# William-gregory/SeaIceExtentForecasting

Hardware: NVIDIA B200
Metric: retrospective forecasts/sec (network+GPR) (higher is better)
Workload: dtype f64

## Files before the change

### seaiceextentforecasting_b200/csrc/gp.cu

```cuda
#include "common.cuh"

namespace {

constexpr int GT = 256;
constexpr int MAXN = 64;
constexpr int LDS = MAXN + 1;

__device__ const double kTheta[5] = {1.495585217958292e-002, 2.539398330063230e-001, 9.504178996162932e-001,
                                     2.097847961257068e+000, 4.25};
__device__ const double kCoeff[5] = {1.1102230246251565e-16 * 100800.0, 1.1102230246251565e-16 * 10059033600.0,
                                     1.1102230246251565e-16 * 4487938430976000.0,
                                     1.1102230246251565e-16 * 5914384781877411840000.0,
                                     1.1102230246251565e-16 * 113250775606021113483283660800000000.0};
__device__ const double kB3[4] = {120., 60., 12., 1.};
__device__ const double kB5[6] = {30240., 15120., 3360., 420., 30., 1.};
__device__ const double kB7[8] = {17297280., 8648640., 1995840., 277200., 25200., 1512., 56., 1.};
__device__ const double kB9[10] = {17643225600., 8821612800., 2075673600., 302702400., 30270240.,
                                   2162160., 110880., 3960., 90., 1.};
__device__ const double kB13[14] = {64764752532480000., 32382376266240000., 7771770303897600., 1187353796428800.,
                                    129060195264000., 10559470521600., 670442572800., 33522128640., 1323241920.,
                                    40840800., 960960., 16380., 182., 1.};

__device__ unsigned long long g_gp_phase[16];
#ifdef SIE_GP_TIMERS
#define GP_TICK(i) do { if (threadIdx.x == 0) { const long long t__ = clock64(); atomicAdd(&g_gp_phase[i], (unsigned long long)(t__ - gp_t_last)); gp_t_last = t__; } } while (0)
#else
#define GP_TICK(i) do { } while (0)
#endif
constexpr int KC = 16;
constexpr int LDA_S = 20;
constexpr int LDB_S = 68;
constexpr int PANEL = 16;

struct Smem {
  double As[2][64 * LDA_S];
  double Bs[2][KC * LDB_S];
  union {
    struct {
      double K[MAXN * LDS];
      double W[MAXN * LDS];
    } gp;
    double panel[2 * MAXN * LDS];
  } u;
  double y[MAXN], ya[MAXN], alpha[MAXN], kxs[MAXN], v[MAXN];
  double red[GT / 32];
  int ired[GT / 32];
  int misc[8];
  double dmisc[8];
  int piv[PANEL];
};

__device__ __forceinline__ double block_sum(double v, Smem& sm) {
#pragma unroll
  for (int o = 16; o > 0; o >>= 1) v += __shfl_xor_sync(0xffffffffu, v, o);
  __syncthreads();
  if ((threadIdx.x & 31) == 0) sm.red[threadIdx.x >> 5] = v;
  __syncthreads();
  double r = 0.0;
#pragma unroll
  for (int w = 0; w < GT / 32; ++w) r += sm.red[w];
  return r;
}
__device__ __forceinline__ double block_max(double v, Smem& sm) {
#pragma unroll
  for (int o = 16; o > 0; o >>= 1) v = fmax(v, __shfl_xor_sync(0xffffffffu, v, o));
  __syncthreads();
  if ((threadIdx.x & 31) == 0) sm.red[threadIdx.x >> 5] = v;
  __syncthreads();
  double r = sm.red[0];
#pragma unroll
  for (int w = 1; w < GT / 32; ++w) r = fmax(r, sm.red[w]);
  return r;
}

__device__ __forceinline__ void dmma884(double& c0, double& c1, double a, double b) {
  asm volatile("mma.sync.aligned.m8n8k4.row.col.f64.f64.f64.f64 {%0,%1}, {%2}, {%3}, {%0,%1};"
               : "+d"(c0), "+d"(c1)
               : "d"(a), "d"(b));
}

__device__ __noinline__ void cta_gemm(double* __restrict__ Cm, int ldc, const double* __restrict__ A, int lda,
                         const double* __restrict__ Bm, int ldb, int m, int k, int n2, Smem& sm, int mode = 0) {
  if (m <= 0 || n2 <= 0 || k <= 0) { __syncthreads(); return; }
  const int tid = threadIdx.x, lane = tid & 31, warp = tid >> 5;
  const int wr = warp >> 1, wc = warp & 1;
  const int tm = (m + 63) >> 6, tn = (n2 + 63) >> 6, kc = (k + KC - 1) / KC;
  const int nsteps = tm * tn * kc;
  const int ar = tid >> 2, ak = (tid & 3) * 4;
  const int bk = tid >> 4, bc = (tid & 15) * 4;
  double ra[4], rb[4];
  auto gload = [&](int step) {
    const int t = step / kc, c = step - t * kc;
    const int ti = t / tn, tj = t - ti * tn;
    const int gr = ti * 64 + ar, gk = c * KC + ak;
    const double* pa = A + (size_t)gr * lda + gk;
#pragma unroll
    for (int q = 0; q < 4; ++q) ra[q] = (gr < m && gk + q < k) ? pa[q] : 0.0;
    const int gkb = c * KC + bk, gc = tj * 64 + bc;
    const double* pb = Bm + (size_t)gkb * ldb + gc;
#pragma unroll
    for (int q = 0; q < 4; ++q) rb[q] = (gkb < k && gc + q < n2) ? pb[q] : 0.0;
  };
  auto spark = [&](int bufi) {
    double* as = sm.As[bufi] + ar * LDA_S + ak;
    double* bs = sm.Bs[bufi] + bk * LDB_S + bc;
    *reinterpret_cast<double2*>(as) = make_double2(ra[0], ra[1]);
    *reinterpret_cast<double2*>(as + 2) = make_double2(ra[2], ra[3]);
    *reinterpret_cast<double2*>(bs) = make_double2(rb[0], rb[1]);
    *reinterpret_cast<double2*>(bs + 2) = make_double2(rb[2], rb[3]);
  };
  double acc[2][4][2];
  gload(0);
  spark(0);
  __syncthreads();
  for (int step = 0; step < nsteps; ++step) {
    const int bufi = step & 1;
    const int t = step / kc, c = step - t * kc;
    if (step + 1 < nsteps) gload(step + 1);
    if (c == 0) {
#pragma unroll
      for (int i = 0; i < 2; ++i)
#pragma unroll
        for (int jj = 0; jj < 4; ++jj) acc[i][jj][0] = acc[i][jj][1] = 0.0;
    }
    const double* as = sm.As[bufi] + (wr * 16 + (lane >> 2)) * LDA_S + (lane & 3);
    const double* bs = sm.Bs[bufi] + (lane & 3) * LDB_S + wc * 32 + (lane >> 2);
#pragma unroll
    for (int ks = 0; ks < KC / 4; ++ks) {
      double af[2], bf[4];
#pragma unroll
      for (int i = 0; i < 2; ++i) af[i] = as[i * 8 * LDA_S + ks * 4];
#pragma unroll
      for (int jj = 0; jj < 4; ++jj) bf[jj] = bs[ks * 4 * LDB_S + jj * 8];
#pragma unroll
      for (int i = 0; i < 2; ++i)
#pragma unroll
        for (int jj = 0; jj < 4; ++jj) dmma884(acc[i][jj][0], acc[i][jj][1], af[i], bf[jj]);
    }
    if (c == kc - 1) {
      const int ti = t / tn, tj = t - ti * tn;
#pragma unroll
      for (int i = 0; i < 2; ++i) {
        const int gr = ti * 64 + wr * 16 + i * 8 + (lane >> 2);
        if (gr >= m) continue;
#pragma unroll
        for (int jj = 0; jj < 4; ++jj) {
          const int gc = tj * 64 + wc * 32 + jj * 8 + 2 * (lane & 3);
          double* pc = Cm + (size_t)gr * ldc + gc;
          if (gc < n2) pc[0] = mode ? pc[0] - acc[i][jj][0] : acc[i][jj][0];
          if (gc + 1 < n2) pc[1] = mode ? pc[1] - acc[i][jj][1] : acc[i][jj][1];
        }
      }
    }
    if (step + 1 < nsteps) spark(bufi ^ 1);
    __syncthreads();
  }
}

__device__ __noinline__ double cta_norm1(const double* __restrict__ A, int ld, int np_, Smem& sm) {
  double best = 0.0;
  for (int j = threadIdx.x; j < np_; j += GT) {
    double s = 0.0;
    for (int i = 0; i < np_; ++i) s += fabs(A[(size_t)i * ld + j]);
    best = fmax(best, s);
  }
  return block_max(best, sm);
}

__device__ __noinline__ double cta_absnorm_power(const double* __restrict__ A, int ld, int np_, double scale, int p,
                                    double* __restrict__ v0, double* __restrict__ v1, Smem& sm) {
  const int parts = (np_ <= GT / 8) ? 8 : (np_ <= GT / 4) ? 4 : (np_ <= GT / 2) ? 2 : 1;
  double* part = &sm.As[0][0];
  const int jc = threadIdx.x % np_, sl = threadIdx.x / np_;
  for (int j = threadIdx.x; j < np_; j += GT) v0[j] = 1.0;
  __syncthreads();
  double* src = v0;
  double* dst = v1;
  for (int it = 0; it < p; ++it) {
    if (parts > 1) {
      if (sl < parts) {
        double s = 0.0;
#pragma unroll 4
        for (int i = sl; i < np_; i += parts) s = fma(scale * fabs(A[(size_t)i * ld + jc]), src[i], s);
        part[sl * np_ + jc] = s;
      }
      __syncthreads();
      if (threadIdx.x < np_) {
        double s = part[threadIdx.x];
        for (int q = 1; q < parts; ++q) s += part[q * np_ + threadIdx.x];
        dst[threadIdx.x] = s;
      }
    } else {
      for (int j = threadIdx.x; j < np_; j += GT) {
        double s = 0.0;
#pragma unroll 4
        for (int i = 0; i < np_; ++i) s = fma(scale * fabs(A[(size_t)i * ld + j]), src[i], s);
        dst[j] = s;
      }
    }
    __syncthreads();
    double* t = src; src = dst; dst = t;
  }
  double best = 0.0;
  for (int j = threadIdx.x; j < np_; j += GT) best = fmax(best, src[j]);
  return block_max(best, sm);
}

__device__ __forceinline__ int ell_of(double t, double normA, int idx, int m) {
  if (!(t > 0.0)) return 0;
  const double val = ceil(log2(t / normA / kCoeff[idx]) / (double)(2 * m));
  if (val != val) return 1 << 20;
  if (val > 1.0e6) return 1 << 20;
  return val > 0.0 ? (int)val : 0;
}

__device__ __noinline__ void cta_lincomb(double* __restrict__ dst, int ld, int np_, double cI, const double* P1, double c1,
                            const double* P2, double c2, const double* P3, double c3, const double* add) {
#pragma unroll 4
  for (int idx = threadIdx.x; idx < np_ * np_; idx += GT) {
    const int i = idx / np_, jj = idx - i * np_;
    const size_t o = (size_t)i * ld + jj;
    double v = (i == jj) ? cI : 0.0;
    if (P1) v += c1 * P1[o];
    if (P2) v += c2 * P2[o];
    if (P3) v += c3 * P3[o];
    if (add) v += add[o];
    dst[o] = v;
  }
  __syncthreads();
}

__device__ __noinline__ void cta_lu_solve(double* __restrict__ P, double* __restrict__ Q, int ld, int np_, Smem& sm) {
  const int tid = threadIdx.x;
  double* pan = sm.u.panel;
  for (int k0 = 0; k0 < np_; k0 += PANEL) {
    const int kb = min(PANEL, np_ - k0);
    const int rows = np_ - k0;
    for (int idx = tid; idx < rows * PANEL; idx += GT) {
      const int r = idx / PANEL, c = idx - r * PANEL;
      pan[idx] = (c < kb) ? P[(size_t)(k0 + r) * ld + k0 + c] : 0.0;
    }
    __syncthreads();
    for (int c = 0; c < kb; ++c) {
      double bv = -1.0; int bi = c;
      for (int r = c + tid; r < rows; r += GT) {
        const double a = fabs(pan[r * PANEL + c]);
        if (a > bv) { bv = a; bi = r; }
      }
#pragma unroll
      for (int o = 16; o > 0; o >>= 1) {
        const double ov = __shfl_xor_sync(0xffffffffu, bv, o);
        const int oi = __shfl_xor_sync(0xffffffffu, bi, o);
        if (ov > bv || (ov == bv && oi < bi)) { bv = ov; bi = oi; }
      }
      if ((tid & 31) == 0) { sm.red[tid >> 5] = bv; sm.ired[tid >> 5] = bi; }
      __syncthreads();
      bv = sm.red[0]; bi = sm.ired[0];
#pragma unroll
      for (int w = 1; w < GT / 32; ++w)
        if (sm.red[w] > bv || (sm.red[w] == bv && sm.ired[w] < bi)) { bv = sm.red[w]; bi = sm.ired[w]; }
      if (tid == 0) sm.piv[c] = bi;
      if (bi != c && tid < PANEL) {
        const double t = pan[c * PANEL + tid]; pan[c * PANEL + tid] = pan[bi * PANEL + tid]; pan[bi * PANEL + tid] = t;
      }
      __syncthreads();
      const double inv = 1.0 / pan[c * PANEL + c];
      for (int r = c + 1 + tid; r < rows; r += GT) pan[r * PANEL + c] *= inv;
      __syncthreads();
      const int cw = kb - c - 1;
      if (cw > 0) {
        for (int idx = tid; idx < (rows - c - 1) * cw; idx += GT) {
          const int r = c + 1 + idx / cw, c2 = c + 1 + idx % cw;
          pan[r * PANEL + c2] = fma(-pan[r * PANEL + c], pan[c * PANEL + c2], pan[r * PANEL + c2]);
        }
      }
      __syncthreads();
    }
    for (int idx = tid; idx < rows * kb; idx += GT) {
      const int r = idx / kb, c = idx - r * kb;
      P[(size_t)(k0 + r) * ld + k0 + c] = pan[r * PANEL + c];
    }
    const int rightw = np_ - k0 - kb;
    for (int col = tid; col < rightw + np_; col += GT) {
      double* base = (col < rightw) ? P + (k0 + kb + col) : Q + (col - rightw);
      for (int c = 0; c < kb; ++c) {
        const int pr = sm.piv[c];
        if (pr != c) {
          const double t = base[(size_t)(k0 + c) * ld]; base[(size_t)(k0 + c) * ld] = base[(size_t)(k0 + pr) * ld];
          base[(size_t)(k0 + pr) * ld] = t;
        }
      }
      double x[PANEL];
#pragma unroll
      for (int c = 0; c < PANEL; ++c) x[c] = (c < kb) ? base[(size_t)(k0 + c) * ld] : 0.0;
#pragma unroll
      for (int c = 1; c < PANEL; ++c) {
        if (c < kb) {
          double sacc = x[c];
#pragma unroll
          for (int d = 0; d < PANEL; ++d)
            if (d < c) sacc = fma(-pan[c * PANEL + d], x[d], sacc);
          x[c] = sacc;
        }
      }
#pragma unroll
      for (int c = 0; c < PANEL; ++c)
        if (c < kb) base[(size_t)(k0 + c) * ld] = x[c];
    }
    __syncthreads();
    const int below = np_ - k0 - kb;
    if (below > 0) {
      const double* L21 = P + (size_t)(k0 + kb) * ld + k0;
      cta_gemm(P + (size_t)(k0 + kb) * ld + k0 + kb, ld, L21, ld, P + (size_t)k0 * ld + k0 + kb, ld, below, kb, rightw,
               sm, 1);
      cta_gemm(Q + (size_t)(k0 + kb) * ld, ld, L21, ld, Q + (size_t)k0 * ld, ld, below, kb, np_, sm, 1);
    }
  }
  const int nblk = (np_ + PANEL - 1) / PANEL;
  for (int b = nblk - 1; b >= 0; --b) {
    const int k0 = b * PANEL, kb = min(PANEL, np_ - k0);
    for (int idx = tid; idx < PANEL * PANEL; idx += GT) {
      const int r = idx / PANEL, c = idx - r * PANEL;
      pan[idx] = (r < kb && c < kb) ? P[(size_t)(k0 + r) * ld + k0 + c] : 0.0;
    }
    __syncthreads();
    for (int col = tid; col < np_; col += GT) {
      double x[PANEL];
#pragma unroll
      for (int c = 0; c < PANEL; ++c) x[c] = (c < kb) ? Q[(size_t)(k0 + c) * ld + col] : 0.0;
#pragma unroll
      for (int c = PANEL - 1; c >= 0; --c) {
        if (c < kb) {
          double sacc = x[c];
#pragma unroll
          for (int d = 0; d < PANEL; ++d)
            if (d > c && d < kb) sacc = fma(-pan[c * PANEL + d], x[d], sacc);
          x[c] = sacc / pan[c * PANEL + c];
        }
      }
#pragma unroll
      for (int c = 0; c < PANEL; ++c)
        if (c < kb) Q[(size_t)(k0 + c) * ld + col] = x[c];
    }
    __syncthreads();
    if (k0 > 0) cta_gemm(Q, ld, P + k0, ld, Q + (size_t)k0 * ld, ld, k0, kb, np_, sm, 1);
  }
}

__device__ __noinline__ double* cta_expm(double** buf, int ld, int np_, double* v0, double* v1, int* m_out, int* s_out,
                            Smem& sm) {
  double* A = buf[1]; double* A2 = buf[2]; double* A4 = buf[3]; double* A6 = buf[4];
  double* B5 = buf[5]; double* B6 = buf[6]; double* B7 = buf[7]; double* B8 = buf[8];
  long long gp_t_last = clock64();
  (void)gp_t_last;
  cta_gemm(A2, ld, A, ld, A, ld, np_, np_, np_, sm);
  cta_gemm(A4, ld, A2, ld, A2, ld, np_, np_, np_, sm);
  cta_gemm(A6, ld, A4, ld, A2, ld, np_, np_, np_, sm);
  const double normA = cta_norm1(A, ld, np_, sm);
  const double d4 = pow(cta_norm1(A4, ld, np_, sm), 0.25);
  const double d6 = pow(cta_norm1(A6, ld, np_, sm), 1.0 / 6.0);
  const double eta0 = fmax(d4, d6);
  GP_TICK(1);
  int m = 0, s = 0;
  if (eta0 < kTheta[0] && ell_of(cta_absnorm_power(A, ld, np_, 1.0, 7, v0, v1, sm), normA, 0, 3) == 0) m = 3;
  if (!m && eta0 < kTheta[1] && ell_of(cta_absnorm_power(A, ld, np_, 1.0, 11, v0, v1, sm), normA, 1, 5) == 0) m = 5;
  double d8 = 0.0, eta2 = 0.0;
  if (!m) {
    cta_gemm(B5, ld, A4, ld, A4, ld, np_, np_, np_, sm);
    d8 = pow(cta_norm1(B5, ld, np_, sm), 0.125);
    eta2 = fmax(d6, d8);
    if (eta2 < kTheta[2] && ell_of(cta_absnorm_power(A, ld, np_, 1.0, 15, v0, v1, sm), normA, 2, 7) == 0) m = 7;
    if (!m && eta2 < kTheta[3] && ell_of(cta_absnorm_power(A, ld, np_, 1.0, 19, v0, v1, sm), normA, 3, 9) == 0) m = 9;
  }
  GP_TICK(2);
  double* U = B7; double* V = B8;
  if (m == 3) {
    cta_lincomb(B5, ld, np_, kB3[1], A2, kB3[3], nullptr, 0, nullptr, 0, nullptr);
    cta_gemm(U, ld, A, ld, B5, ld, np_, np_, np_, sm);
    cta_lincomb(V, ld, np_, kB3[0], A2, kB3[2], nullptr, 0, nullptr, 0, nullptr);
  } else if (m == 5) {
    cta_lincomb(B5, ld, np_, kB5[1], A4, kB5[5], A2, kB5[3], nullptr, 0, nullptr);
    cta_gemm(U, ld, A, ld, B5, ld, np_, np_, np_, sm);
    cta_lincomb(V, ld, np_, kB5[0], A4, kB5[4], A2, kB5[2], nullptr, 0, nullptr);
  } else if (m == 7) {
    cta_lincomb(B5, ld, np_, kB7[1], A6, kB7[7], A4, kB7[5], A2, kB7[3], nullptr);
    cta_gemm(U, ld, A, ld, B5, ld, np_, np_, np_, sm);
    cta_lincomb(V, ld, np_, kB7[0], A6, kB7[6], A4, kB7[4], A2, kB7[2], nullptr);
  } else if (m == 9) {
    cta_lincomb(B6, ld, np_, kB9[1], A6, kB9[7], A4, kB9[5], A2, kB9[3], nullptr);
    for (int idx = threadIdx.x; idx < np_ * np_; idx += GT) {
      const int i = idx / np_, jj = idx - i * np_; const size_t o = (size_t)i * ld + jj;
      B6[o] += kB9[9] * B5[o];
    }
    __syncthreads();
    cta_gemm(U, ld, A, ld, B6, ld, np_, np_, np_, sm);
    cta_lincomb(V, ld, np_, kB9[0], A6, kB9[6], A4, kB9[4], A2, kB9[2], nullptr);
    for (int idx = threadIdx.x; idx < np_ * np_; idx += GT) {
      const int i = idx / np_, jj = idx - i * np_; const size_t o = (size_t)i * ld + jj;
      V[o] += kB9[8] * B5[o];
    }
    __syncthreads();
  } else {
    m = 13;
    cta_gemm(B6, ld, A4, ld, A6, ld, np_, np_, np_, sm);
    const double d10 = pow(cta_norm1(B6, ld, np_, sm), 0.1);
    const double eta3 = fmax(d8, d10), eta4 = fmin(eta2, eta3);
    double sv = ceil(log2(eta4 / kTheta[4]));
    s = (sv > 0.0) ? (int)sv : 0;
    if (!(sv == sv) || sv > 2000.0) s = 2000;
    const double sc = ldexp(1.0, -s);
    GP_TICK(2);
    s += ell_of(cta_absnorm_power(A, ld, np_, sc, 27, v0, v1, sm), normA * sc, 4, 13);
    GP_TICK(3);
    if (s > 2000) s = 2000;
    const double s1 = ldexp(1.0, -s), s2 = ldexp(1.0, -2 * s), s4 = ldexp(1.0, -4 * s), s6 = ldexp(1.0, -6 * s);
#pragma unroll 2
    for (int idx = threadIdx.x; idx < np_ * np_; idx += GT) {
      const int i = idx / np_, jj = idx - i * np_; const size_t o = (size_t)i * ld + jj;
      A[o] *= s1; A2[o] *= s2; A4[o] *= s4; A6[o] *= s6;
    }
    __syncthreads();
    cta_lincomb(B5, ld, np_, 0.0, A6, kB13[13], A4, kB13[11], A2, kB13[9], nullptr);
    cta_gemm(B6, ld, A6, ld, B5, ld, np_, np_, np_, sm);
    cta_lincomb(B5, ld, np_, kB13[1], A6, kB13[7], A4, kB13[5], A2, kB13[3], B6);
    cta_gemm(U, ld, A, ld, B5, ld, np_, np_, np_, sm);
    cta_lincomb(B5, ld, np_, 0.0, A6, kB13[12], A4, kB13[10], A2, kB13[8], nullptr);
    cta_gemm(B6, ld, A6, ld, B5, ld, np_, np_, np_, sm);
    cta_lincomb(V, ld, np_, kB13[0], A6, kB13[6], A4, kB13[4], A2, kB13[2], B6);
  }
  GP_TICK(4);
#pragma unroll 4
  for (int idx = threadIdx.x; idx < np_ * np_; idx += GT) {
    const int i = idx / np_, jj = idx - i * np_; const size_t o = (size_t)i * ld + jj;
    const double u = U[o], vv = V[o];
    B5[o] = vv - u; B6[o] = vv + u;
  }
  __syncthreads();
  cta_lu_solve(B5, B6, ld, np_, sm);
  GP_TICK(5);
  double* Xc = B6; double* Xn = B7;
  for (int it = 0; it < s; ++it) {
    cta_gemm(Xn, ld, Xc, ld, Xc, ld, np_, np_, np_, sm);
    double* t = Xc; Xc = Xn; Xn = t;
  }
  GP_TICK(6);
  *m_out = m; *s_out = s;
  return Xc;
}

__device__ __noinline__ int cta_cholesky(double* K, int n, Smem& sm) {
  const int tid = threadIdx.x;
  for (int k = 0; k < n; ++k) {
    const double d = K[k * LDS + k];
    if (!(d > 0.0)) return k + 1;
    const double r = sqrt(d);
    __syncthreads();
    if (tid == 0) K[k * LDS + k] = r;
    for (int i = k + 1 + tid; i < n; i += GT) K[i * LDS + k] /= r;
    __syncthreads();
    const int rem = n - k - 1;
    for (int idx = tid; idx < rem * rem; idx += GT) {
      const int a = idx / rem, b = idx - a * rem;
      if (b <= a) {
        const int i = k + 1 + a, jj = k + 1 + b;
        K[i * LDS + jj] = fma(-K[i * LDS + k], K[jj * LDS + k], K[i * LDS + jj]);
      }
    }
    __syncthreads();
  }
  return 0;
}
__device__ __forceinline__ void warp_fwd_solve(const double* L, int n, const double* b, double* tmp, int lane) {
  for (int i = 0; i < n; ++i) {
    double s = 0.0;
    for (int c = lane; c < i; c += 32) s = fma(L[i * LDS + c], tmp[c], s);
#pragma unroll
    for (int o = 16; o > 0; o >>= 1) s += __shfl_xor_sync(0xffffffffu, s, o);
    if (lane == 0) tmp[i] = (b[i] - s) / L[i * LDS + i];
    __syncwarp();
  }
}
__device__ __forceinline__ void warp_bwd_solve(const double* L, int n, const double* tmp, double* x, int lane) {
  for (int i = n - 1; i >= 0; --i) {
    double s = 0.0;
    for (int c = i + 1 + lane; c < n; c += 32) s = fma(L[c * LDS + i], x[c], s);
#pragma unroll
    for (int o = 16; o > 0; o >>= 1) s += __shfl_xor_sync(0xffffffffu, s, o);
    if (lane == 0) x[i] = (tmp[i] - s) / L[i * LDS + i];
    __syncwarp();
  }
}
__device__ void cta_chol_solve(const double* L, int n, const double* b, double* x, double* tmp) {
  if (threadIdx.x < 32) {
    warp_fwd_solve(L, n, b, tmp, threadIdx.x);
    warp_bwd_solve(L, n, tmp, x, threadIdx.x);
  }
  __syncthreads();
}

__device__ __forceinline__ int warp_cholesky(double* K, int n, int ldw, int lane) {
  for (int k = 0; k < n; ++k) {
    const double d = K[k * ldw + k];
    if (!(d > 0.0)) return k + 1;
    const double r = sqrt(d);
    __syncwarp();
    if (lane == 0) K[k * ldw + k] = r;
    for (int i = k + 1 + lane; i < n; i += 32) K[i * ldw + k] /= r;
    __syncwarp();
    for (int i = k + 1 + lane; i < n; i += 32) {
      const double aik = K[i * ldw + k];
      for (int jj = k + 1; jj <= i; ++jj) K[i * ldw + jj] = fma(-aik, K[jj * ldw + k], K[i * ldw + jj]);
    }
    __syncwarp();
  }
  return 0;
}
__device__ __forceinline__ void warp_fwd_solve_ld(const double* L, int n, int ldw, const double* b, double* tmp, int lane) {
  for (int i = 0; i < n; ++i) {
    double s = 0.0;
    for (int c = lane; c < i; c += 32) s = fma(L[i * ldw + c], tmp[c], s);
#pragma unroll
    for (int o = 16; o > 0; o >>= 1) s += __shfl_xor_sync(0xffffffffu, s, o);
    if (lane == 0) tmp[i] = (b[i] - s) / L[i * ldw + i];
    __syncwarp();
  }
}
__device__ __forceinline__ void warp_bwd_solve_ld(const double* L, int n, int ldw, const double* tmp, double* x, int lane) {
  for (int i = n - 1; i >= 0; --i) {
    double s = 0.0;
    for (int c = i + 1 + lane; c < n; c += 32) s = fma(L[c * ldw + i], x[c], s);
#pragma unroll
    for (int o = 16; o > 0; o >>= 1) s += __shfl_xor_sync(0xffffffffu, s, o);
    if (lane == 0) x[i] = (tmp[i] - s) / L[i * ldw + i];
    __syncwarp();
  }
}

__device__ void warp_sigma_fit(const double* __restrict__ W, const double* __restrict__ y, const double* __restrict__ kxs_raw,
                               double kss_raw, const double* __restrict__ G1raw, int n, double sig, double* Kw, double* vec,
                               SieGpResult& res, long long clk_start, SieGpResult* outp) {
  const int lane = threadIdx.x & 31;
  const int ldw = n | 1;
  double* ya = vec; double* alpha = vec + MAXN; double* kxs = vec + 2 * MAXN; double* v = vec + 3 * MAXN;
  res.fmean = res.fvar = res.sigma_f = res.nlml = res.g_ell = res.g_sig = sie_nan();
  res.info = 0;
  for (int idx = lane; idx < n * n; idx += 32) {
    const int i = idx / n, jj = idx - i * n;
    Kw[i * ldw + jj] = W[i * LDS + jj] + ((i == jj) ? sig : 0.0);
  }
  __syncwarp();
  int info = warp_cholesky(Kw, n, ldw, lane);
  if (info) { if (lane == 0) { res.info = info; res.cycles_total = clock64() - clk_start; *outp = res; } return; }
  warp_fwd_solve_ld(Kw, n, ldw, y, v, lane);
  warp_bwd_solve_ld(Kw, n, ldw, v, ya, lane);
  double sf = 0.0;
  for (int t = 0; t < n; ++t) sf = fma(y[t], ya[t], sf);
  sf /= (double)n;
  const double sn = sf * sig;
  res.sigma_f = sf;
  __syncwarp();
  for (int idx = lane; idx < n * n; idx += 32) {
    const int i = idx / n, jj = idx - i * n;
    Kw[i * ldw + jj] = sf * W[i * LDS + jj] + ((i == jj) ? sn : 0.0);
  }
  __syncwarp();
  info = warp_cholesky(Kw, n, ldw, lane);
  if (info) { if (lane == 0) { res.info = info; res.cycles_total = clock64() - clk_start; *outp = res; } return; }
  warp_fwd_solve_ld(Kw, n, ldw, y, v, lane);
  warp_bwd_solve_ld(Kw, n, ldw, v, alpha, lane);
  for (int i = lane; i < n; i += 32) kxs[i] = sf * kxs_raw[i];
  __syncwarp();
  const double kss = sf * kss_raw + sn;
  warp_fwd_solve_ld(Kw, n, ldw, kxs, v, lane);
  double vv = 0.0, fm = 0.0, yal = 0.0, ld_sum = 0.0;
  for (int i = lane; i < n; i += 32) {
    vv = fma(v[i], v[i], vv);
    fm = fma(kxs[i], alpha[i], fm);
    yal = fma(y[i], alpha[i], yal);
    ld_sum += log(Kw[i * ldw + i]);
  }
#pragma unroll
  for (int o = 16; o > 0; o >>= 1) {
    vv += __shfl_xor_sync(0xffffffffu, vv, o);
    fm += __shfl_xor_sync(0xffffffffu, fm, o);
    yal += __shfl_xor_sync(0xffffffffu, yal, o);
    ld_sum += __shfl_xor_sync(0xffffffffu, ld_sum, o);
  }
  res.fmean = fm; res.fvar = kss - vv;
  res.nlml = yal / 2 + ld_sum + n * log(2 * 3.141592653589793238462643383279502884) / 2;
  if (G1raw) {
    for (int which = 0; which < 2; ++which) {
      auto dK = [&](int i, int jj) -> double {
        return which == 0 ? sf * G1raw[i * LDS + jj] + ((i == jj) ? sn : 0.0) : sf * W[i * LDS + jj] + ((i == jj) ? sf : 0.0);
      };
      double quad = 0.0;
      for (int idx = lane; idx < n * n; idx += 32) {
        const int i = idx / n, jj = idx - i * n;
        quad = fma(alpha[i] * dK(i, jj), alpha[jj], quad);
      }
      double tr = 0.0;
      for (int jj = lane; jj < n; jj += 32) {
        double col[MAXN];
        for (int i = 0; i < n; ++i) {
          double sacc = dK(i, jj);
          for (int c = 0; c < i; ++c) sacc = fma(-Kw[i * ldw + c], col[c], sacc);
          col[i] = sacc / Kw[i * ldw + i];
        }
        for (int i = n - 1; i >= jj; --i) {
          double sacc = col[i];
          for (int c = i + 1; c < n; ++c) sacc = fma(-Kw[c * ldw + i], col[c], sacc);
          col[i] = sacc / Kw[i * ldw + i];
        }
        tr += col[jj];
      }
#pragma unroll
      for (int o = 16; o > 0; o >>= 1) {
        quad += __shfl_xor_sync(0xffffffffu, quad, o);
        tr += __shfl_xor_sync(0xffffffffu, tr, o);
      }
      const double gval = tr / 2 - quad / 2;
      if (which == 0) res.g_ell = gval; else res.g_sig = gval;
    }
  }
  if (lane == 0) { res.cycles_total = clock64() - clk_start; *outp = res; }
}

__global__ void __launch_bounds__(GT, 2)
k_gp_forecast(const SieGpProblem* __restrict__ prob, int P, const double* __restrict__ y_all,
              const double* __restrict__ anom_sic, const int32_t* __restrict__ n_areas_sic, int ma_sic, int ts_sic,
              const double* __restrict__ anom_sst, const int32_t* __restrict__ n_areas_sst, int ma_sst, int ts_sst,
              int max_pred, SieGpResult* __restrict__ out, unsigned char* __restrict__ scratch, size_t per_cta,
              const int32_t* __restrict__ order, int* __restrict__ queue, const double* __restrict__ sig_grid,
              int n_sig) {
  const int ns = sig_grid ? n_sig : 1;
  extern __shared__ __align__(16) unsigned char smraw[];
  Smem& sm = *reinterpret_cast<Smem*>(smraw);
  const int tid = threadIdx.x;
  const int ld = max_pred;
  unsigned char* sp = scratch + (size_t)blockIdx.x * per_cta;
  double* buf[9];
  for (int i = 0; i < 9; ++i) buf[i] = reinterpret_cast<double*>(sp) + (size_t)i * ld * ld;
  double* Xg = reinterpret_cast<double*>(sp) + (size_t)9 * ld * ld;
  double* XE = Xg + (size_t)MAXN * ld;
  double* XM = XE + (size_t)MAXN * ld;
  double* v0 = XM + (size_t)MAXN * ld;
  double* v1 = v0 + ld;
  double* colm = v1 + ld;
  double* Gg = colm + ld;
  int* sel = reinterpret_cast<int*>(Gg + MAXN * LDS);

  while (true) {
    __syncthreads();
    if (tid == 0) sm.misc[7] = atomicAdd(queue, 1);
    __syncthreads();
    const int qi = sm.misc[7];
    if (qi >= P) break;
    const int p = order ? order[qi] : qi;
    const SieGpProblem pr = prob[p];
    const int n = pr.n;
    SieGpResult res;
    res.fmean = res.fvar = res.sigma_f = res.nlml = res.g_ell = res.g_sig = sie_nan();
    res.n_pred = 0; res.expm_m = 0; res.expm_s = 0; res.info = 0;
    res.cycles_total = 0; res.cycles_expm = 0;
    const long long clk_start = clock64();
    long long gp_t_last = clk_start;
    (void)gp_t_last;
    __syncthreads();
    if (n < 2 || n + 1 > MAXN) {
      if (tid == 0) { res.info = -2; for (int k = 0; k < ns; ++k) out[(size_t)p * ns + k] = res; }
      continue;
    }
    const int na1 = n_areas_sic[pr.job_sic];
    const int na2 = (pr.job_sst >= 0) ? n_areas_sst[pr.job_sst] : 0;
    const double* s1 = anom_sic + (size_t)pr.job_sic * ma_sic * ts_sic;
    const double* s2 = (pr.job_sst >= 0) ? anom_sst + (size_t)pr.job_sst * ma_sst * ts_sst : nullptr;
    for (int t = tid; t < n; t += GT) sm.y[t] = y_all[pr.y_off + t];
    __syncthreads();
    double ymean = 0.0;
    for (int t = 0; t < n; ++t) ymean += sm.y[t];
    ymean /= (double)n;
    double ynorm = 0.0;
    for (int t = 0; t < n; ++t) { const double d = sm.y[t] - ymean; ynorm = fma(d, d, ynorm); }
    ynorm = sqrt(ynorm);
    if (tid == 0) sm.misc[0] = 0;
    __syncthreads();
    for (int c0 = 0; c0 < na1 + na2; c0 += GT) {
      const int c = c0 + tid;
      int flag = 0;
      if (c < na1 + na2) {
        const bool sst = c >= na1;
        const double* x = sst ? s2 + (size_t)(c - na1) * ts_sst : s1 + (size_t)c * ts_sic;
        double xm = 0.0;
        for (int t = 0; t < n; ++t) xm += x[t];
        xm /= (double)n;
        double xn = 0.0, dot = 0.0;
        for (int t = 0; t < n; ++t) { const double d = x[t] - xm; xn = fma(d, d, xn); dot = fma(d, sm.y[t] - ymean, dot); }
        double r = dot / (sqrt(xn) * ynorm);
        if (r == r) r = fmax(-1.0, fmin(1.0, r));
        if (sst) flag = (r < 0.0) ? 2 : 0;
        else if (pr.rule == 1) flag = 1;
        else if (pr.rule == 0) flag = (r > 0.0) ? 1 : 0;
        else flag = (r > 0.0 && r > pr.r_sel) ? 1 : 0;
      }
      const unsigned bal = __ballot_sync(0xffffffffu, flag != 0);
      const int lane = tid & 31, w = tid >> 5;
      if (lane == 0) sm.ired[w] = __popc(bal);
      __syncthreads();
      int off = sm.misc[0];
      for (int i = 0; i < w; ++i) off += sm.ired[i];
      if (flag) {
        const int pos = off + __popc(bal & ((1u << lane) - 1u));
        if (pos < ld) sel[pos] = c | (flag == 2 ? (1 << 30) : 0);
      }
      __syncthreads();
      if (tid == 0) { int tot = 0; for (int i = 0; i < GT / 32; ++i) tot += sm.ired[i]; sm.misc[0] += tot; }
// ... 370 lines not shown
```

Measured before the change: 67420.

## Exploit symmetry in matrix squares, reuse power iterations, restructure LU pivoting

Squares of the (symmetric) matrix in the Padé expm path are computed only on upper block tiles and mirrored, which cuts MMA work for A^2, A^4 and A^8. The abs-norm power iteration now resumes from the previous iteration count instead of restarting for each Padé degree test. The panel LU fuses pivot search for the next column into the rank-1 update, dropping one barrier per column, and applies row swaps as a precomputed permutation instead of sequential swaps. These changes add complexity and assume A is exactly symmetric. The mirroring pass is an extra global-memory sweep.

```diff
diff --git a/seaiceextentforecasting_b200/csrc/gp.cu b/seaiceextentforecasting_b200/csrc/gp.cu
--- a/seaiceextentforecasting_b200/csrc/gp.cu
+++ b/seaiceextentforecasting_b200/csrc/gp.cu
@@ -48,6 +48,7 @@
   int misc[8];
   double dmisc[8];
   int piv[PANEL];
+  int src_top[PANEL], mv_dst[PANEL], mv_src[PANEL], mv_pos[2 * PANEL], mv_cur[2 * PANEL];
 };
 
 __device__ __forceinline__ double block_sum(double v, Smem& sm) {
@@ -79,19 +80,33 @@
                : "d"(a), "d"(b));
 }
 
+enum GemmMode {
+  GEMM_SET = 0,
+  GEMM_SUB = 1,
+  GEMM_SYM_SQUARE = 2,
+};
 __device__ __noinline__ void cta_gemm(double* __restrict__ Cm, int ldc, const double* __restrict__ A, int lda,
-                         const double* __restrict__ Bm, int ldb, int m, int k, int n2, Smem& sm, int mode = 0) {
+                         const double* __restrict__ Bm, int ldb, int m, int k, int n2, Smem& sm,
+                         GemmMode mode = GEMM_SET) {
   if (m <= 0 || n2 <= 0 || k <= 0) { __syncthreads(); return; }
   const int tid = threadIdx.x, lane = tid & 31, warp = tid >> 5;
   const int wr = warp >> 1, wc = warp & 1;
+  const bool sub = mode == GEMM_SUB, upper = mode == GEMM_SYM_SQUARE;
   const int tm = (m + 63) >> 6, tn = (n2 + 63) >> 6, kc = (k + KC - 1) / KC;
-  const int nsteps = tm * tn * kc;
+  const int nsteps = (upper ? tm * (tm + 1) / 2 : tm * tn) * kc;
+  auto tile = [&](int t, int& ti, int& tj) {
+    if (!upper) { ti = t / tn; tj = t - ti * tn; return; }
+    ti = 0;
+    while (t >= tm - ti) { t -= tm - ti; ++ti; }
+    tj = ti + t;
+  };
   const int ar = tid >> 2, ak = (tid & 3) * 4;
   const int bk = tid >> 4, bc = (tid & 15) * 4;
   double ra[4], rb[4];
   auto gload = [&](int step) {
     const int t = step / kc, c = step - t * kc;
-    const int ti = t / tn, tj = t - ti * tn;
+    int ti, tj;
+    tile(t, ti, tj);
     const int gr = ti * 64 + ar, gk = c * KC + ak;
     const double* pa = A + (size_t)gr * lda + gk;
 #pragma unroll
@@ -138,7 +153,8 @@
         for (int jj = 0; jj < 4; ++jj) dmma884(acc[i][jj][0], acc[i][jj][1], af[i], bf[jj]);
     }
     if (c == kc - 1) {
-      const int ti = t / tn, tj = t - ti * tn;
+      int ti, tj;
+      tile(t, ti, tj);
 #pragma unroll
       for (int i = 0; i < 2; ++i) {
         const int gr = ti * 64 + wr * 16 + i * 8 + (lane >> 2);
@@ -147,12 +163,19 @@
         for (int jj = 0; jj < 4; ++jj) {
           const int gc = tj * 64 + wc * 32 + jj * 8 + 2 * (lane & 3);
           double* pc = Cm + (size_t)gr * ldc + gc;
-          if (gc < n2) pc[0] = mode ? pc[0] - acc[i][jj][0] : acc[i][jj][0];
-          if (gc + 1 < n2) pc[1] = mode ? pc[1] - acc[i][jj][1] : acc[i][jj][1];
+          if (gc < n2) pc[0] = sub ? pc[0] - acc[i][jj][0] : acc[i][jj][0];
+          if (gc + 1 < n2) pc[1] = sub ? pc[1] - acc[i][jj][1] : acc[i][jj][1];
         }
       }
     }
     if (step + 1 < nsteps) spark(bufi ^ 1);
+    __syncthreads();
+  }
+  if (mode == GEMM_SYM_SQUARE && tm > 1) {
+    for (int idx = tid; idx < m * m; idx += GT) {
+      const int i = idx / m, jj = idx - i * m;
+      if ((i >> 6) > (jj >> 6)) Cm[(size_t)i * ldc + jj] = Cm[(size_t)jj * ldc + i];
+    }
     __syncthreads();
   }
 }
@@ -168,15 +191,17 @@
 }
 
 __device__ __noinline__ double cta_absnorm_power(const double* __restrict__ A, int ld, int np_, double scale, int p,
-                                    double* __restrict__ v0, double* __restrict__ v1, Smem& sm) {
+                                    int& done, double* __restrict__ v0, double* __restrict__ v1, Smem& sm) {
   const int parts = (np_ <= GT / 8) ? 8 : (np_ <= GT / 4) ? 4 : (np_ <= GT / 2) ? 2 : 1;
   double* part = &sm.As[0][0];
   const int jc = threadIdx.x % np_, sl = threadIdx.x / np_;
-  for (int j = threadIdx.x; j < np_; j += GT) v0[j] = 1.0;
-  __syncthreads();
-  double* src = v0;
-  double* dst = v1;
-  for (int it = 0; it < p; ++it) {
+  if (done == 0) {
+    for (int j = threadIdx.x; j < np_; j += GT) v0[j] = 1.0;
+    __syncthreads();
+  }
+  double* src = (done & 1) ? v1 : v0;
+  double* dst = (done & 1) ? v0 : v1;
+  for (int it = done; it < p; ++it) {
     if (parts > 1) {
       if (sl < parts) {
         double s = 0.0;
@@ -201,6 +226,7 @@
     __syncthreads();
     double* t = src; src = dst; dst = t;
   }
+  done = p;
   double best = 0.0;
   for (int j = threadIdx.x; j < np_; j += GT) best = fmax(best, src[j]);
   return block_max(best, sm);
@@ -233,6 +259,15 @@
 __device__ __noinline__ void cta_lu_solve(double* __restrict__ P, double* __restrict__ Q, int ld, int np_, Smem& sm) {
   const int tid = threadIdx.x;
   double* pan = sm.u.panel;
+  auto pivot_partial = [&](double bv, int bi) {
+#pragma unroll
+    for (int o = 16; o > 0; o >>= 1) {
+      const double ov = __shfl_xor_sync(0xffffffffu, bv, o);
+      const int oi = __shfl_xor_sync(0xffffffffu, bi, o);
+      if (ov > bv || (ov == bv && oi < bi)) { bv = ov; bi = oi; }
+    }
+    if ((tid & 31) == 0) { sm.red[tid >> 5] = bv; sm.ired[tid >> 5] = bi; }
+  };
   for (int k0 = 0; k0 < np_; k0 += PANEL) {
     const int kb = min(PANEL, np_ - k0);
     const int rows = np_ - k0;
@@ -241,21 +276,17 @@
       pan[idx] = (c < kb) ? P[(size_t)(k0 + r) * ld + k0 + c] : 0.0;
     }
     __syncthreads();
+    {
+      double bv = -1.0; int bi = 0;
+      for (int r = tid; r < rows; r += GT) {
+        const double a = fabs(pan[r * PANEL]);
+        if (a > bv) { bv = a; bi = r; }
+      }
+      pivot_partial(bv, bi);
+    }
+    __syncthreads();
     for (int c = 0; c < kb; ++c) {
-      double bv = -1.0; int bi = c;
-      for (int r = c + tid; r < rows; r += GT) {
-        const double a = fabs(pan[r * PANEL + c]);
-        if (a > bv) { bv = a; bi = r; }
-      }
-#pragma unroll
-      for (int o = 16; o > 0; o >>= 1) {
-        const double ov = __shfl_xor_sync(0xffffffffu, bv, o);
-        const int oi = __shfl_xor_sync(0xffffffffu, bi, o);
-        if (ov > bv || (ov == bv && oi < bi)) { bv = ov; bi = oi; }
-      }
-      if ((tid & 31) == 0) { sm.red[tid >> 5] = bv; sm.ired[tid >> 5] = bi; }
-      __syncthreads();
-      bv = sm.red[0]; bi = sm.ired[0];
+      double bv = sm.red[0]; int bi = sm.ired[0];
 #pragma unroll
       for (int w = 1; w < GT / 32; ++w)
         if (sm.red[w] > bv || (sm.red[w] == bv && sm.ired[w] < bi)) { bv = sm.red[w]; bi = sm.ired[w]; }
@@ -265,34 +296,57 @@
       }
       __syncthreads();
       const double inv = 1.0 / pan[c * PANEL + c];
-      for (int r = c + 1 + tid; r < rows; r += GT) pan[r * PANEL + c] *= inv;
+      double nv = -1.0; int ni = c + 1;
+      for (int r = c + 1 + tid; r < rows; r += GT) {
+        const double l = pan[r * PANEL + c] * inv;
+        pan[r * PANEL + c] = l;
+#pragma unroll
+        for (int c2 = 1; c2 < PANEL; ++c2)
+          if (c2 > c && c2 < kb) pan[r * PANEL + c2] = fma(-l, pan[c * PANEL + c2], pan[r * PANEL + c2]);
+        if (c + 1 < kb) {
+          const double a = fabs(pan[r * PANEL + c + 1]);
+          if (a > nv) { nv = a; ni = r; }
+        }
+      }
+      if (c + 1 < kb) pivot_partial(nv, ni);
       __syncthreads();
-      const int cw = kb - c - 1;
-      if (cw > 0) {
-        for (int idx = tid; idx < (rows - c - 1) * cw; idx += GT) {
-          const int r = c + 1 + idx / cw, c2 = c + 1 + idx % cw;
-          pan[r * PANEL + c2] = fma(-pan[r * PANEL + c], pan[c * PANEL + c2], pan[r * PANEL + c2]);
-        }
-      }
-      __syncthreads();
+    }
+    if (tid == 0) {
+      int* pos = sm.mv_pos; int* cur = sm.mv_cur; int n = 0;
+      auto slot = [&](int r) {
+        for (int q = 0; q < n; ++q) if (pos[q] == r) return q;
+        pos[n] = r; cur[n] = r; return n++;
+      };
+      for (int c = 0; c < kb; ++c) {
+        const int pr = sm.piv[c];
+        if (pr != c) { const int x = slot(c), y = slot(pr); const int t = cur[x]; cur[x] = cur[y]; cur[y] = t; }
+      }
+      for (int c = 0; c < PANEL; ++c) sm.src_top[c] = c;
+      int nm = 0;
+      for (int q = 0; q < n; ++q) {
+        if (pos[q] < kb) sm.src_top[pos[q]] = cur[q];
+        else if (cur[q] != pos[q]) { sm.mv_dst[nm] = pos[q]; sm.mv_src[nm] = cur[q]; ++nm; }
+      }
+      sm.misc[6] = nm;
     }
     for (int idx = tid; idx < rows * kb; idx += GT) {
       const int r = idx / kb, c = idx - r * kb;
       P[(size_t)(k0 + r) * ld + k0 + c] = pan[r * PANEL + c];
     }
+    __syncthreads();
+    const int nm = sm.misc[6];
     const int rightw = np_ - k0 - kb;
     for (int col = tid; col < rightw + np_; col += GT) {
       double* base = (col < rightw) ? P + (k0 + kb + col) : Q + (col - rightw);
-      for (int c = 0; c < kb; ++c) {
-        const int pr = sm.piv[c];
-        if (pr != c) {
-          const double t = base[(size_t)(k0 + c) * ld]; base[(size_t)(k0 + c) * ld] = base[(size_t)(k0 + pr) * ld];
-          base[(size_t)(k0 + pr) * ld] = t;
-        }
-      }
-      double x[PANEL];
-#pragma unroll
-      for (int c = 0; c < PANEL; ++c) x[c] = (c < kb) ? base[(size_t)(k0 + c) * ld] : 0.0;
+      double x[PANEL], mv[PANEL];
+#pragma unroll
+      for (int c = 0; c < PANEL; ++c) x[c] = (c < kb) ? base[(size_t)(k0 + sm.src_top[c]) * ld] : 0.0;
+#pragma unroll
+      for (int q = 0; q < PANEL; ++q)
+        if (q < nm) mv[q] = base[(size_t)(k0 + sm.mv_src[q]) * ld];
+#pragma unroll
+      for (int q = 0; q < PANEL; ++q)
+        if (q < nm) base[(size_t)(k0 + sm.mv_dst[q]) * ld] = mv[q];
 #pragma unroll
       for (int c = 1; c < PANEL; ++c) {
         if (c < kb) {
@@ -312,8 +366,8 @@
     if (below > 0) {
       const double* L21 = P + (size_t)(k0 + kb) * ld + k0;
       cta_gemm(P + (size_t)(k0 + kb) * ld + k0 + kb, ld, L21, ld, P + (size_t)k0 * ld + k0 + kb, ld, below, kb, rightw,
-               sm, 1);
-      cta_gemm(Q + (size_t)(k0 + kb) * ld, ld, L21, ld, Q + (size_t)k0 * ld, ld, below, kb, np_, sm, 1);
+               sm, GEMM_SUB);
+      cta_gemm(Q + (size_t)(k0 + kb) * ld, ld, L21, ld, Q + (size_t)k0 * ld, ld, below, kb, np_, sm, GEMM_SUB);
     }
   }
   const int nblk = (np_ + PANEL - 1) / PANEL;
@@ -343,7 +397,7 @@
         if (c < kb) Q[(size_t)(k0 + c) * ld + col] = x[c];
     }
     __syncthreads();
-    if (k0 > 0) cta_gemm(Q, ld, P + k0, ld, Q + (size_t)k0 * ld, ld, k0, kb, np_, sm, 1);
+    if (k0 > 0) cta_gemm(Q, ld, P + k0, ld, Q + (size_t)k0 * ld, ld, k0, kb, np_, sm, GEMM_SUB);
   }
 }
 
@@ -353,8 +407,8 @@
   double* B5 = buf[5]; double* B6 = buf[6]; double* B7 = buf[7]; double* B8 = buf[8];
   long long gp_t_last = clock64();
   (void)gp_t_last;
-  cta_gemm(A2, ld, A, ld, A, ld, np_, np_, np_, sm);
-  cta_gemm(A4, ld, A2, ld, A2, ld, np_, np_, np_, sm);
+  cta_gemm(A2, ld, A, ld, A, ld, np_, np_, np_, sm, GEMM_SYM_SQUARE);
+  cta_gemm(A4, ld, A2, ld, A2, ld, np_, np_, np_, sm, GEMM_SYM_SQUARE);
   cta_gemm(A6, ld, A4, ld, A2, ld, np_, np_, np_, sm);
   const double normA = cta_norm1(A, ld, np_, sm);
   const double d4 = pow(cta_norm1(A4, ld, np_, sm), 0.25);
@@ -362,15 +416,16 @@
   const double eta0 = fmax(d4, d6);
   GP_TICK(1);
   int m = 0, s = 0;
-  if (eta0 < kTheta[0] && ell_of(cta_absnorm_power(A, ld, np_, 1.0, 7, v0, v1, sm), normA, 0, 3) == 0) m = 3;
-  if (!m && eta0 < kTheta[1] && ell_of(cta_absnorm_power(A, ld, np_, 1.0, 11, v0, v1, sm), normA, 1, 5) == 0) m = 5;
+  int pw = 0;
+  if (eta0 < kTheta[0] && ell_of(cta_absnorm_power(A, ld, np_, 1.0, 7, pw, v0, v1, sm), normA, 0, 3) == 0) m = 3;
+  if (!m && eta0 < kTheta[1] && ell_of(cta_absnorm_power(A, ld, np_, 1.0, 11, pw, v0, v1, sm), normA, 1, 5) == 0) m = 5;
   double d8 = 0.0, eta2 = 0.0;
   if (!m) {
-    cta_gemm(B5, ld, A4, ld, A4, ld, np_, np_, np_, sm);
+    cta_gemm(B5, ld, A4, ld, A4, ld, np_, np_, np_, sm, GEMM_SYM_SQUARE);
     d8 = pow(cta_norm1(B5, ld, np_, sm), 0.125);
     eta2 = fmax(d6, d8);
-    if (eta2 < kTheta[2] && ell_of(cta_absnorm_power(A, ld, np_, 1.0, 15, v0, v1, sm), normA, 2, 7) == 0) m = 7;
-    if (!m && eta2 < kTheta[3] && ell_of(cta_absnorm_power(A, ld, np_, 1.0, 19, v0, v1, sm), normA, 3, 9) == 0) m = 9;
+    if (eta2 < kTheta[2] && ell_of(cta_absnorm_power(A, ld, np_, 1.0, 15, pw, v0, v1, sm), normA, 2, 7) == 0) m = 7;
+    if (!m && eta2 < kTheta[3] && ell_of(cta_absnorm_power(A, ld, np_, 1.0, 19, pw, v0, v1, sm), normA, 3, 9) == 0) m = 9;
   }
   GP_TICK(2);
   double* U = B7; double* V = B8;
@@ -410,7 +465,8 @@
     if (!(sv == sv) || sv > 2000.0) s = 2000;
     const double sc = ldexp(1.0, -s);
     GP_TICK(2);
-    s += ell_of(cta_absnorm_power(A, ld, np_, sc, 27, v0, v1, sm), normA * sc, 4, 13);
+    int pw13 = 0;
+    s += ell_of(cta_absnorm_power(A, ld, np_, sc, 27, pw13, v0, v1, sm), normA * sc, 4, 13);
     GP_TICK(3);
     if (s > 2000) s = 2000;
     const double s1 = ldexp(1.0, -s), s2 = ldexp(1.0, -2 * s), s4 = ldexp(1.0, -4 * s), s6 = ldexp(1.0, -6 * s);
```

Result: slower. 66670, median of 6 (-1.1%).
